# sglang-npu/DeepGEMM_Ascend

Hardware: AMD Instinct MI355X
Metric: fp8 TFLOPS + % MFMA peak, 4096^3 block-scaled GEMM; grouped-GEMM tok/s at 1/2/4/8 GPU (higher is better)
Workload: dtype bf16

## Files before the change

### deepgemm_ascend_amd/__init__.py

```python
from ._lib import DGAError, DGALibraryError, Platform, Problem, Tiling, build, lib
from .api import (
    CONFIG_FIELDS,
    bbit_params,
    bench_params_fill,
    catlass_dynamic_matmul,
    combine_tokens,
    combine_tokens_weight_grad,
    copy_rows,
    copy_rows2,
    gather_per_token_cast_to_fp8_transposed,
    gemm_fp8_fp8_bf16_nt,
    gemm_fp8_fp8_fp32_nt,
    tiling_check_fp32_out,
    tiling_fp32_out,
    tiling_check_wgrad,
    tiling_wgrad,
    wgrad_gemm_fp8_fp8_fp32_nt,
    k_grouped_wgrad_gemm_fp8_fp8_fp32_nt,
    tiling_check_k_grouped_wgrad,
    tiling_k_grouped_wgrad,
    gemm_fp8_loop_clock,
    get_bench_config,
    get_best_config,
    infer_dtype,
    infer_shape,
    get_m_alignment_for_contiguous_layout,
    m_grouped_gemm_fp8_fp8_bf16_nt_contiguous,
    m_grouped_gemm_fp8_fp8_bf16_nt_masked,
    m_grouped_gemm_fp8_fp8_bf16_nt_masked_indexed,
    mfma_ceiling,
    per_block_cast_to_fp8,
    per_block_cast_to_fp8_transposed,
    per_token_cast_to_fp8,
    per_token_cast_to_fp8_transposed,
    platform_ascend910b,
    predict_time_us,
    route_slots,
    router_topk,
    router_topk_backward,
    route_tokens,
    predictor_load,
    predictor_loaded,
    predictor_unload,
    release_scratch,
    select_kernel_with_predictor,
    select_tiling_strategy,
    silu_and_mul_per_token_cast_to_fp8,
    silu_and_mul_per_token_cast_to_fp8_transposed,
    silu_and_mul_backward_per_token_cast_to_fp8,
    platform_mi355x,
    run_mmad_bench,
    run_mmad_custom,
    run_mmad_rtc,
    select_kernel,
    tiling,
    tiling_check,
    tiling_cache_clear,
    tiling_cache_open,
    tiling_cache_size,
    workspace_bytes,
)
# ... 3 lines not shown
```

### deepgemm_ascend_amd/_lib.py

```python
from __future__ import annotations

import ctypes
import os
import subprocess
from ctypes import POINTER, c_char_p, c_float, c_int, c_int32, c_int64, c_size_t, c_uint8, c_uint16, c_uint32, c_uint64, c_void_p
from pathlib import Path

_PKG = Path(__file__).resolve().parent
LIB_PATH = _PKG / "libdga_hip.so"


class DGALibraryError(RuntimeError):
    pass


class DGAError(RuntimeError):

    def __init__(self, status: int, where: str, detail: str = ""):
        self.status = status
        msg = f"{where}: status {status} ({status_string(status)})"
        if detail:
            msg += f" {detail}"
        super().__init__(msg)

# ... 109 lines not shown
    "dga_cast_to_fp8_128x128": (c_int, [c_void_p, c_int, c_int64, c_int64, c_void_p, c_void_p, c_void_p]),
    "dga_cast_to_fp8_1x128_ld": (c_int, [c_void_p, c_int, c_int64, c_int64, c_void_p, c_int64, c_void_p, c_void_p]),
    "dga_cast_to_fp8_128x128_ld": (c_int, [c_void_p, c_int, c_int64, c_int64, c_void_p, c_int64, c_void_p, c_void_p]),
    "dga_cast_to_fp8_1x128_ex": (c_int, [c_void_p, c_int, c_int64, c_int64, c_void_p, c_int64, c_void_p, c_int, c_void_p]),
    "dga_cast_to_fp8_128x128_ex": (c_int, [c_void_p, c_int, c_int64, c_int64, c_void_p, c_int64, c_void_p, c_int, c_void_p]),
    "dga_silu_mul_cast_to_fp8_1x128": (c_int, [c_void_p, c_int, c_int64, c_int64, c_int64, c_void_p, c_void_p, c_void_p, c_void_p, c_int,
                                       c_void_p]),
    "dga_silu_mul_bwd_cast_to_fp8_1x128": (c_int, [c_void_p, c_void_p, c_int, c_int64, c_int64, c_int64, c_void_p, c_void_p, c_void_p,
                                           c_void_p, c_void_p, c_int, c_void_p]),
    "dga_cast_to_fp8_1x128_transposed": (c_int, [c_void_p, c_int, c_int64, c_int64, c_int64, c_void_p, c_void_p, c_void_p, c_int64,
                                         c_void_p, c_void_p, c_void_p, c_int, c_void_p]),
    "dga_silu_mul_cast_to_fp8_1x128_transposed": (c_int, [c_void_p, c_int, c_int64, c_int64, c_int64, c_void_p, c_void_p, c_void_p, c_int64,
                                                  c_void_p, c_void_p, c_void_p, c_int, c_void_p]),
    "dga_cast_to_fp8_128x128_transposed": (c_int, [c_void_p, c_int, c_int64, c_int64, c_int64, c_void_p, c_void_p, c_void_p, c_void_p, c_int,
                                           c_void_p]),
    "dga_gather_cast_to_fp8_1x128_transposed": (c_int, [c_void_p, c_int, c_int64, c_int64, c_void_p, c_int64, c_void_p, c_int64, c_int64,
                                                c_void_p, c_void_p, c_int64, c_void_p, c_void_p, c_void_p, c_int, c_void_p]),
    "dga_combine_rows": (c_int, [c_void_p, c_int, c_int64, c_int64, c_void_p, c_void_p, c_int64, c_int64, c_void_p, c_int, c_void_p]),
    "dga_combine_rows_weight_grad": (c_int, [c_void_p, c_void_p, c_int, c_int64, c_int64, c_void_p, c_int64, c_int64, c_void_p, c_void_p]),
    "dga_router_topk": (c_int, [c_void_p, c_int, c_int64, c_int64, c_int64, c_int, c_void_p, c_int64, c_int64, c_int, c_float, c_void_p, c_void_p,
                                c_void_p, c_void_p]),
    "dga_router_topk_backward": (c_int, [c_void_p, c_void_p, c_void_p, c_int64, c_int64, c_int64, c_int, c_int, c_float, c_void_p, c_int,
                                         c_void_p]),
    "dga_catlass_dynamic_matmul_workspace_bytes": (c_size_t, [c_int, c_int, c_int, c_void_p, c_void_p]),
    "dga_catlass_dynamic_matmul": (c_int, [c_void_p, c_void_p, c_void_p, c_int, c_int, c_int, c_int, c_void_p, c_size_t,
                                           c_void_p]),
    "dga_get_best_config": (c_int, [c_uint32] * 4 + [POINTER(c_uint32)]),
    "dga_get_bench_config": (c_int, [c_uint32] * 9 + [POINTER(c_uint32)]),
    "dga_bench_params_fill": (c_int, [c_uint32] * 3 + [POINTER(c_int32)]),
    "dga_bbit_params": (c_int, [c_uint32] * 9 + [POINTER(c_uint32)]),
    "dga_run_mmad_rtc": (c_int, [c_void_p, c_void_p, c_void_p, c_int, c_int, c_int, c_int, c_int, c_void_p]),
    "dga_run_mmad_bench": (c_int, [c_void_p, c_void_p, c_void_p, c_int, c_int, c_int, c_int, POINTER(c_int32),
                                   c_void_p]),
    "dga_mmad_workspace_bytes": (c_size_t, [c_int, c_int, c_int, c_int, c_void_p]),
    "dga_run_mmad_rtc_ws": (c_int, [c_void_p, c_void_p, c_void_p, c_int, c_int, c_int, c_int, c_int, c_void_p, c_size_t,
                                    c_void_p]),
    "dga_run_mmad_bench_ws": (c_int, [c_void_p, c_void_p, c_void_p, c_int, c_int, c_int, c_int, POINTER(c_int32),
                                      c_void_p, c_size_t, c_void_p]),
    "dga_route_tokens": (c_int, [c_void_p, c_int64, c_int, c_void_p, c_void_p, c_void_p]),
    "dga_route_slots": (c_int, [c_void_p, c_int64, c_int64, c_int, c_int, c_int, c_int, c_int, c_void_p, c_int, c_void_p,
                                c_void_p, c_int64, c_void_p, c_void_p, c_int64, c_void_p]),
    "dga_m_grouped_gemm_fp8_fp8_bf16_nt_masked_indexed": (c_int, [c_void_p, c_int64, c_void_p, c_int64, c_void_p, c_void_p,
                                                                  c_void_p, c_int64, c_void_p, c_int64, c_void_p, c_int,
                                                                  c_int, c_int, c_int, c_int, POINTER(Tiling), c_void_p,
                                                                  c_size_t, c_void_p]),
    "dga_copy_rows2": (c_int, [c_void_p, c_int64, c_void_p, c_int64, c_int64, c_void_p, c_int64, c_void_p, c_int64, c_int64,
# ... 81 lines not shown
```

### deepgemm_ascend_amd/api.py

```python
from __future__ import annotations

import ctypes
import os
from typing import Optional, Sequence, Tuple

import torch

from . import _lib
from ._lib import DGAError, Platform, Problem, Tiling

_FP8 = getattr(torch, "float8_e4m3fn", None)


_raw_stream = getattr(torch._C, "_cuda_getCurrentRawStream", None)


def _stream_of(index: int) -> int:
    if _raw_stream is not None:
        return _raw_stream(index)
    return torch.cuda.current_stream(index).cuda_stream


def _stream_ptr(t: torch.Tensor) -> int:
    if t.is_cuda:
# ... 614 lines not shown
    if masked_m.dtype != torch.int32 or masked_m.dim() != 1 or masked_m.shape[0] != g:
        _fail("masked_m must be int32 [G]")
    if not (a.is_contiguous() and b.is_contiguous() and sfa.is_contiguous() and sfb.is_contiguous() and out.is_contiguous() and
            masked_m.is_contiguous()):
        _fail("operands must be contiguous")
    expected_m = int(expected_m)
    with _device_guard(a, b, sfa, sfb, out, masked_m):
        index = out.device.index
        if tiling_ is None:
            tiling_ = _planned(index, mmax, n, k, g, expected_m, False, strict, policy)
        else:
            tiling_ = _with_policy(tiling_, strict, policy)
        stream = _stream_of(index)
        ws_ptr, ws_bytes = _workspace(tiling_, out.device, stream)
        rc = _lib.lib().dga_m_grouped_gemm_fp8_fp8_bf16_nt_masked(
            a.data_ptr(), sfa.data_ptr(), b.data_ptr(), sfb.data_ptr(), out.data_ptr(), masked_m.data_ptr(),
            g, mmax, n, k, expected_m, ctypes.byref(tiling_), ws_ptr, ws_bytes, stream)
        if rc:
            _lib.check(rc, "m_grouped_gemm_fp8_fp8_bf16_nt_masked")
        if sync:
            torch.cuda.current_stream(out.device).synchronize()


def m_grouped_gemm_fp8_fp8_bf16_nt_masked_indexed(a_rows: torch.Tensor, sfa_src: torch.Tensor, sfa_byte_offset: int,
                                                  sfa_ld: int, rhs, out_rows: torch.Tensor, row_index: torch.Tensor,
                                                  masked_m: torch.Tensor, m_max: int, expected_m: int = 0,
                                                  tiling_: Optional[Tiling] = None, sync: bool = False,
                                                  strict: bool = False, policy: Optional[str] = None) -> None:
    b, sfb = rhs
    _fp8_bytes(b); _fp8_bytes(a_rows)
    _require(a_rows.dim() == 2 and a_rows.stride(1) == 1 and out_rows.dim() == 2 and out_rows.stride(1) == 1, "2-D row tensors")
    g, n, k = b.shape
    rows, lda = a_rows.shape[0], a_rows.stride(0)
    kb, nb = (k + 127) // 128, (n + 127) // 128
    _require(a_rows.shape[1] >= k and out_rows.shape[1] >= n and out_rows.dtype == torch.bfloat16, "row widths")
    _require(out_rows.shape[0] >= rows, "out_rows must have a row for every source row")
    _require(tuple(sfb.shape) == (g, nb, kb) and sfb.dtype == torch.float32, f"sfb must be [{g},{nb},{kb}] f32")
    _require(row_index.dtype == torch.int64 and row_index.numel() >= g * m_max and row_index.is_contiguous(), "row_index int64[G*m_max]")
    _require(masked_m.dtype == torch.int32 and tuple(masked_m.shape) == (g,), "masked_m must be int32 [G]")
    _require(sfa_byte_offset % 4 == 0 and sfa_ld >= kb, "scale rows must be float-aligned")
    _require(sfa_src.dim() == 2 and sfa_src.stride(1) == 1 and sfa_src.dtype in (torch.float32, torch.uint8),
             "sfa_src must be a 2-D float32 (or uint8 payload) row tensor with unit inner stride")
    _require(sfa_src.stride(0) * sfa_src.element_size() == 4 * sfa_ld, "sfa_ld must be sfa_src's row stride in floats")
    _require(sfa_src.data_ptr() % 4 == 0 and sfa_src.shape[0] >= rows and
             sfa_byte_offset + 4 * kb <= sfa_src.shape[1] * sfa_src.element_size(),
             "sfa_src must hold ceil(K/128) floats at sfa_byte_offset of each of the source's rows")
# ... 532 lines not shown
```

### deepgemm_ascend_amd/csrc/dga_fp8_menu.hpp

```cpp
#pragma once
#include "dga_internal.hpp"
#include "gemm_fp8_kernel.hpp"

namespace dga {

template <class Cfg, int PP, bool CLK = false>
int launch_cfg(const GemmParams &p, hipStream_t stream);

#define DGA_MENU_A(X) X(256, 256, 4, 2, 2, 0) X(256, 256, 4, 2, 2, 1) X(256, 256, 4, 2, 2, 2)
#define DGA_MENU_B(X)                                                                                              \
    X(128, 256, 2, 2, 2, 2) X(256, 128, 4, 1, 2, 2) X(128, 128, 2, 2, 2, 2) X(64, 256, 1, 4, 2, 2) X(128, 256, 2, 4, 2, 2)
#define DGA_MENU_C(X)                                                                                              \
    X(128, 256, 2, 2, 2, 0) X(256, 128, 4, 1, 2, 0) X(128, 128, 2, 2, 2, 0) X(64, 256, 1, 4, 2, 0) X(64, 128, 1, 4, 2, 0) \
    X(128, 256, 2, 4, 2, 0) X(128, 256, 2, 4, 3, 0) X(128, 256, 2, 2, 3, 0) X(128, 128, 2, 2, 3, 0) X(64, 256, 1, 4, 3, 0) \
    X(32, 256, 1, 4, 2, 0) X(32, 128, 1, 4, 2, 0) X(16, 256, 1, 4, 2, 0) X(16, 128, 1, 4, 2, 0)                        \
    X(64, 128, 1, 4, 3, 0) X(32, 256, 1, 4, 3, 0) X(32, 128, 1, 4, 3, 0) X(16, 256, 1, 4, 3, 0) X(16, 128, 1, 4, 3, 0)
#define DGA_MENU_LC(X) X(128, 256, 2, 2, 3, 0) X(128, 128, 2, 2, 3, 0) X(64, 256, 1, 4, 3, 0) X(64, 128, 1, 4, 3, 0) X(16, 128, 1, 4, 3, 0)
#define DGA_MENU_CLK(X) X(256, 256, 4, 2, 2, 2)
#define DGA_MENU_CLK_LC(X) X(128, 256, 2, 2, 3, 0)

#define DGA_MENU_EXTERN(BM, BN, WM, WN, ST, PP) \
    extern template int launch_cfg<GemmCfg<BM, BN, WM, WN, ST>, PP, false>(const GemmParams &, hipStream_t);
#define DGA_MENU_EXTERN_CLK(BM, BN, WM, WN, ST, PP) \
    extern template int launch_cfg<GemmCfg<BM, BN, WM, WN, ST>, PP, true>(const GemmParams &, hipStream_t);
// ... 20 lines not shown
#define DGA_MENU_EXTERN_BX(BM, BN, WM, WN, ST, PP) \
    extern template int launch_bf16x<GemmCfg<BM, BN, WM, WN, ST>>(const GemmParams &, hipStream_t);
DGA_MENU_BX(DGA_MENU_EXTERN_BX)
template <class Cfg>
int launch_bf16x_f32(const GemmParams &p, hipStream_t stream);
#define DGA_MENU_EXTERN_BX_F32(BM, BN, WM, WN, ST, PP) \
    extern template int launch_bf16x_f32<GemmCfg<BM, BN, WM, WN, ST>>(const GemmParams &, hipStream_t);
DGA_MENU_BX(DGA_MENU_EXTERN_BX_F32)
template <class Cfg>
int launch_bf16x_rows(const GemmParams &p, hipStream_t stream);
#define DGA_MENU_EXTERN_BX_ROWS(BM, BN, WM, WN, ST, PP) \
    extern template int launch_bf16x_rows<GemmCfg<BM, BN, WM, WN, ST>>(const GemmParams &, hipStream_t);
DGA_MENU_BX(DGA_MENU_EXTERN_BX_ROWS)

int launch_bf16x_image(const GemmParams &p, int waves, hipStream_t stream);
int launch_bf16x_persistent(const GemmParams &p, Out out, hipStream_t stream);
template <class Cfg>
int launch_bf16x_kgroup(const GemmParams &p, hipStream_t stream);
#define DGA_MENU_EXTERN_BX_KGROUP(BM, BN, WM, WN, ST, PP) \
    extern template int launch_bf16x_kgroup<GemmCfg<BM, BN, WM, WN, ST>>(const GemmParams &, hipStream_t);
DGA_MENU_BX(DGA_MENU_EXTERN_BX_KGROUP)
int launch_bf16x_persistent_kgroup(const GemmParams &p, hipStream_t stream);
int launch_strict_kgroup(const GemmParams &p, int bm, hipStream_t stream);
int launch_bf16x_grouped(const GemmParams &p, hipStream_t stream);

int launch_unaligned(const GemmParams &p, hipStream_t stream);

int launch_wsk(const GemmParams &p, hipStream_t stream);
int launch_wsk_dma(const GemmParams &p, hipStream_t stream, int math = 0, Out out = Out::Bf16);
int wsk_rows(int m);
int wsk_max_ntiles(int m);

int launch_ue8m0(int bm, int bn, bool loaders, bool cont, const GemmParams &p, hipStream_t stream);
int launch_ue8m0_w4(const GemmParams &p, hipStream_t stream);
int launch_bf16u(int bm, int bn, const GemmParams &p, hipStream_t stream);

int launch_streamk(const GemmParams &p, void *ws, size_t ws_bytes, bool ue8m0, hipStream_t stream);
size_t streamk_workspace_bytes();
int launch_bf16x_streamk(const GemmParams &p, void *ws, size_t ws_bytes, hipStream_t stream, Out out = Out::Bf16);
size_t bx_streamk_workspace_bytes();
int coresident_workgroups(hipStream_t stream);
int launch_bf16x_dsk(const GemmParams &p, int splits, void *ws, size_t ws_bytes, hipStream_t stream, Out out = Out::Bf16);
int bx_dsk_splits(int64_t tiles, int kb, int want, int cus);
size_t bx_dsk_workspace_bytes(int64_t tiles, int splits);

int launch_cont_persistent(const GemmParams &p, hipStream_t stream);

// ... 2 lines not shown
```

### deepgemm_ascend_amd/csrc/dga_internal.hpp

```cpp
#pragma once
#include <hip/hip_runtime_api.h>

#include "dga_hip.h"
#include <cstdint>
#include <cstdlib>

namespace dga {
int record_hip(hipError_t e);
uint32_t device_cus();
int default_policy();
struct Fp8Indexed {
    const int64_t *row_index;
    int64_t lda;
    int64_t sfa_ld;
    int64_t ldc;
    int64_t rows;
};
struct Fp8Strided {
    int64_t lda, ldb;
    int flags;
};
enum class Out { Bf16, F32, F32Rows };
struct Fp8Call {
    const void *a;
// ... 10 lines not shown
    const int32_t *masked_m = nullptr;
    const int32_t *m_indices = nullptr;
    const Fp8Indexed *ix = nullptr;
    const Fp8Strided *sd = nullptr;
    Out kind = Out::Bf16;
    const float *c_in = nullptr;
    unsigned long long *clock_stamps = nullptr;
};
int run_fp8(const Fp8Call &c);
inline int env_int(const char *name, int dflt)
{
    const char *e = std::getenv(name);
    return e ? std::atoi(e) : dflt;
}
int variant_count();
void variant_info(int i, int *bm, int *bn, int *wm, int *wn, int *lds);
int variant_stages(int i);
bool variant_has_loader_waves(int i);
void prefer_loader_waves(dga_tiling_t &t, bool upgrade_plain = true);
int pad_rows(const void *src0, void *dst0, int64_t rows0, const void *src1, void *dst1, int64_t rows1, int64_t src_row_bytes,
             int64_t dst_row_bytes, hipStream_t stream);
int pad_rows_strided(const void *src0, int64_t stride0, void *dst0, int64_t rows0, const void *src1, int64_t stride1, void *dst1,
                     int64_t rows1, int64_t src_row_bytes, int64_t dst_row_bytes, hipStream_t stream);
void apply_tail_split(dga_tiling_t &t, uint32_t cus);
}
```

### deepgemm_ascend_amd/csrc/dga_launch.hip

```cpp
#include <hip/hip_runtime.h>
#include <atomic>
#include <cstdio>
#include <cstdlib>
#include <cstring>
#include <mutex>

#include "dga_hip.h"
#include "dga_internal.hpp"
#include "dga_fp8_menu_impl.hpp"
#include "gemm_fp8_aux_kernels.hpp"

namespace dga {

static std::atomic<int> g_last_hip_error{0};
int record_hip(hipError_t e)
{
    if (e != hipSuccess) {
        g_last_hip_error.store(static_cast<int>(e));
        return DGA_E_HIP;
    }
    return DGA_OK;
}
uint32_t device_cus()
{
// ... 426 lines not shown
        if (tail > 0 && tail * 2 <= cus && main_tiles > 0 && vq && vq->bm == 64 && vq->bn == 128) {
            GemmParams pm = p;
            pm.launch_tiles = main_tiles;
            rc = launch_bf16x_persistent(pm, c.kind, c.stream);
            if (rc == DGA_E_TILING) rc = vx->launch[form](pm, c.stream);
            if (rc != DGA_OK) return rc;
            GemmParams pt = p;
            pt.tail_begin = main_tiles;
            pt.tail_sub = 2;
            pt.launch_tiles = tail * 4;
            return vq->launch[form](pt, c.stream);
        }
    }
    const int64_t tiles = static_cast<int64_t>(p.groups) * p.tiles_m * p.tiles_n, cus = static_cast<int64_t>(device_cus());
    if (t.kernelSerial == DGA_KERNEL_STREAMK_ONE_LAUNCH && vx->bm == 128 && vx->bn == 256 && dense && c.kind != Out::F32Rows) {
        const size_t need = bx_streamk_workspace_bytes();
        if (uint8_t *sk_ws = carve(need)) {
            rc = launch_bf16x_streamk(p, sk_ws, need, c.stream, c.kind);
            if (rc != DGA_E_TILING) return rc;
        }
    }
    if (vx->bm == 128 && vx->bn == 256 && !c.m_indices && c.kind == Out::Bf16 &&
        (env().bx_grouped >= 0 ? (env().bx_grouped != 0 && c.masked_m) : t.build == DGA_BUILD_BX_GROUPED)) {
        rc = launch_bf16x_grouped(p, c.stream);
        if (rc != DGA_E_TILING) return rc;
    }
    const bool pays = tiles > cus;
    if (vx->bm == 128 && vx->bn == 256 &&
        (env().bx_persist >= 0 ? env().bx_persist != 0 : (t.build == DGA_BUILD_BX_PERSISTENT || (t.build != DGA_BUILD_BX_ONE_TILE && pays)))) {
        rc = launch_bf16x_persistent(p, c.kind, c.stream);
        if (rc != DGA_E_TILING) return rc;
    }
    return vx->launch[form](p, c.stream);
}

static int run_fast(const Fp8Call &c, const dga_tiling_t &t, const Variant *v, bool ue8m0, GemmParams &p, Carver &carve)
{
    const bool dense = c.groups == 1 && !c.masked_m && !c.m_indices && !c.ix;
    const hipStream_t stream = c.stream;
    if (!c.clock_stamps && dense && (env().wsk >= 0 ? env().wsk != 0 : t.kernelSerial == DGA_KERNEL_SPLITK_WORKGROUP)) {
        if (env().wsk_dma >= 0 ? env().wsk_dma != 0 : t.build != DGA_BUILD_WSK_REGISTER) {
            const int rc = launch_wsk_dma(p, stream);
            if (rc != DGA_E_TILING) return rc;
        }
        const int rc = launch_wsk(p, stream);
        if (rc != DGA_E_TILING) return rc;
    }
// ... 374 lines not shown
```

### deepgemm_ascend_amd/csrc/dga_launch_menu_l.hip

```cpp
#include <cstdlib>
#include "dga_fp8_menu_impl.hpp"
#include "gemm_fp8_bf16x_grouped_kernel.hpp"
namespace dga {

template <bool KTAIL, bool BNT, bool STAG, bool IDX = false>
static int launch_bf16x_grouped_one(const GemmParams &p, hipStream_t stream)
{
    typedef GemmCfg<128, 256, 2, 4, 3> Cfg;
    constexpr int kLds = Cfg::LDS_BYTES + (IDX ? 256 * 16 : 0);
    const int64_t tiles = static_cast<int64_t>(p.groups) * p.tiles_m * p.tiles_n;
    const unsigned grid = static_cast<unsigned>(std::min<int64_t>(tiles, device_cus()));
    return launch_kernel<gemm_fp8_bf16x_grouped_kernel<KTAIL, BNT, STAG, IDX>>(grid, Cfg::NT, kLds, stream, p);
}

int launch_bf16x_grouped(const GemmParams &p, hipStream_t stream)
{
    if (p.tail_sub || p.m_indices || p.launch_tiles > 0 || p.splitk > 1 || p.kb_n < 2) return DGA_E_TILING;
    const bool nt = p.b_nt != 0;
#ifdef DGA_BXG_KNOBS
    if (const char *e = std::getenv("DGA_BXG_KNOB"); e && (std::atoi(e) & 2)) {
        if (p.k % 128) return nt ? launch_bf16x_grouped_one<true, true, false>(p, stream) : launch_bf16x_grouped_one<true, false, false>(p, stream);
        return nt ? launch_bf16x_grouped_one<false, true, false>(p, stream) : launch_bf16x_grouped_one<false, false, false>(p, stream);
    }
#endif
    if (p.row_index) {
        if (p.k % 128) return nt ? launch_bf16x_grouped_one<true, true, true, true>(p, stream) : launch_bf16x_grouped_one<true, false, true, true>(p, stream);
        return nt ? launch_bf16x_grouped_one<false, true, true, true>(p, stream) : launch_bf16x_grouped_one<false, false, true, true>(p, stream);
    }
    if (p.k % 128) return nt ? launch_bf16x_grouped_one<true, true, true>(p, stream) : launch_bf16x_grouped_one<true, false, true>(p, stream);
    return nt ? launch_bf16x_grouped_one<false, true, true>(p, stream) : launch_bf16x_grouped_one<false, false, true>(p, stream);
}
}
```

### deepgemm_ascend_amd/csrc/dga_tiling.cpp

```cpp
#include <dlfcn.h>

#include <algorithm>
#include <cmath>
#include <cstdint>
#include <cstdio>
#include <cstdlib>
#include <cstring>
#include <fstream>
#include <map>
#include <mutex>
#include <sstream>
#include <string>
#include <tuple>
#include <vector>

#include "dga_hip.h"
#include "dga_internal.hpp"

namespace dga {
namespace tiling {

inline uint32_t ceil_div(uint32_t a, uint32_t b) { return (a + b - 1) / b; }
inline uint32_t round_up(uint32_t v, uint32_t al) { return ceil_div(v, al) * al; }

// ... 988 lines not shown
}

int dga_tiling_cache_open(const char *csv_path) { return Cache::instance().open(csv_path); }
int dga_tiling_cache_clear(void) { Cache::instance().clear(); return DGA_OK; }
int dga_tiling_cache_size(void) { return Cache::instance().size(); }

size_t dga_workspace_bytes(const dga_tiling_t *tiling)
{
    if (!tiling) return 0;
    size_t bytes = 0;
    auto add = [&](size_t b) { bytes = ((bytes + 255) & ~size_t(255)) + b; };
    const size_t groups = tiling->groups ? tiling->groups : 1;
    if (tiling->k % 16 != 0 && tiling->k > 0) {
        const size_t kp = (static_cast<size_t>(tiling->k) + 127) / 128 * 128;
        add((tiling->contiguous ? 1 : groups) * tiling->m * kp);
        add(groups * tiling->n * kp);
    }
    if (tiling->splitkFactor > 1) add(static_cast<size_t>(tiling->splitkFactor) * tiling->m * tiling->n * 4);
    if (tiling->kernelSerial == DGA_KERNEL_STREAMK_ONE_LAUNCH) add(static_cast<size_t>(dga::device_cus()) * (256 * 256 * 4 + 8) + 256);
    if (tiling->build == DGA_BUILD_BX_DECODE && tiling->splitkFactor > 1) {
        const size_t tiles = (static_cast<size_t>(tiling->m) + 63) / 64 * ((static_cast<size_t>(tiling->n) + 127) / 128);
        add(tiles * (tiling->splitkFactor - 1) * (64 * 128 * 4 + 8) + 256);
    }
    return bytes ? bytes + 256 : 0;
}

const char *dga_status_string(int status)
{
    switch (status) {
        case DGA_OK: return "ok";
        case DGA_E_NULL: return "null pointer";
        case DGA_E_SHAPE: return "shape / rank / layout mismatch";
        case DGA_E_DTYPE: return "dtype mismatch";
        case DGA_E_ALIGN: return "alignment";
        case DGA_E_HIP: return "HIP runtime error";
        case DGA_E_TILING: return "no compiled kernel for this tiling";
        case DGA_E_WORKSPACE: return "workspace too small";
        case DGA_E_IO: return "file error";
        case DGA_E_RANGE: return "value out of range";
        default: return "unknown";
    }
}

int dga_abi_version(void) { return DGA_ABI_VERSION; }

}
// ... 1 lines not shown
```

### deepgemm_ascend_amd/csrc/gemm_fp8_bf16x_grouped_kernel.hpp

```cpp
#pragma once
#include "gemm_fp8_kernel.hpp"

namespace dga {

template <bool KTAIL, bool BNT, bool STAGGER = true, bool INDEXED = false>
__global__ void __launch_bounds__(512) __attribute__((amdgpu_waves_per_eu(2, 2)))
gemm_fp8_bf16x_grouped_kernel(const GemmParams p)
{
    typedef GemmCfg<128, 256, 2, 4, 3> Cfg;
    constexpr int BM = Cfg::kBM, BN = Cfg::kBN, WN = Cfg::kWN, TM = Cfg::TM, TN = Cfg::TN, DNT = Cfg::DNT;
    constexpr int NL = Cfg::LOADS_PER_STAGE, LAGT = 2, RING = 4, NT = Cfg::NT;
    static_assert(Cfg::NT == 512 && DNT == 512 && TM == 4 && TN == 4 && Cfg::SC_ITERS == 1 && Cfg::STAGES == 3, "the grouped schedule");
    typedef __bf16 v8bf __attribute__((ext_vector_type(8)));
    extern __shared__ __attribute__((aligned(16))) uint8_t smem[];

    const int tid = threadIdx.x, lane = tid & 63;
    const int wave = __builtin_amdgcn_readfirstlane(tid >> 6);
    const int wm = wave / WN, wn = wave % WN;
    const int li = lane & 15, kg = lane >> 4;
    const int KB = p.kb_n;

    const int tiles_per_group = p.tiles_m * p.tiles_n;
    const int total = p.groups * tiles_per_group;
    int first = 0, count = total, step = gridDim.x, slot = blockIdx.x;
    if (p.xcd_remap) {
        const int xcd = blockIdx.x & 7, q = total >> 3, r = total & 7;
        first = xcd < r ? xcd * (q + 1) : r * (q + 1) + (xcd - r) * q;
        count = q + (xcd < r ? 1 : 0);
        step = ((int)gridDim.x - xcd + 7) >> 3;
        slot = blockIdx.x >> 3;
    }
    struct Tile { int g, M, m0, n0; };
    typedef const __attribute__((address_space(4))) int32_t *const_i32_ptr;
    const const_i32_ptr masked_m_c = (const_i32_ptr)p.masked_m;
    auto seek = [&](int &local, Tile &t) -> bool {
        for (; local < count; local += step) {
            const int tile = first + local;
            const int g = tile / tiles_per_group;
            const int t_in = tile - g * tiles_per_group;
            const int gm = p.raster_group;
            const int per = gm * p.tiles_n;
            const int band = t_in / per;
            const int row0 = band * gm;
            const int rows = min(p.tiles_m - row0, gm);
            const int loc = t_in - band * per;
            const int tm = row0 + loc % rows, tn = loc / rows;
            const int M = p.masked_m ? min(masked_m_c[g], p.m) : p.m;
            const int m0 = tm * BM;
            if (m0 >= M) continue;
            t.g = g; t.M = M; t.m0 = m0; t.n0 = tn * BN;
            return true;
        }
        return false;
    };

    const uint32_t lds0 = (uint32_t)(uintptr_t)(lptr_t)smem;
    constexpr uint32_t kOutOfRange = 0x80000000u;
    const int a_col = ((tid & 7) ^ swz_a(tid >> 3)) * 16;
    const int b_col = ((tid & 7) ^ swz_b(tid >> 3)) * 16;
    v4i a_rsrc, b_rsrc;
    uint32_t a_voff[Cfg::A_ITERS], b_voff[Cfg::B_ITERS];
    const float *sc_src;
    int kbf = 0;
    bool fill_valid = true;
    constexpr bool indexed = INDEXED;
    static_assert(Cfg::A_ITERS == 2, "partner slot: two A offsets and the scale pointer");
    uint32_t *const pslot = reinterpret_cast<uint32_t *>(smem + Cfg::LDS_BYTES) + (tid & (DNT / 2 - 1)) * 4;
    auto a_off_of = [&](const Tile &t, int it, int td) -> uint32_t {
        const int row = (it * DNT + td) >> 3;
        if (row >= t.M - t.m0) return kOutOfRange;
// ... 337 lines not shown
```

### deepgemm_ascend_amd/csrc/gemm_fp8_kernel.hpp

```cpp
#pragma once
#include "dga_device_common.hpp"
#include "dga_hip.h"

namespace dga {

struct GemmParams {
    const uint8_t *a;
    const float *sfa;
    const uint8_t *b;
    const float *sfb;
    uint16_t *out;
    union {
        const int32_t *masked_m;
        const int32_t *ks;
    };
    const int32_t *m_indices;
    const int64_t *row_index;
    int64_t sfa_ld;
    int64_t a_bytes;
    int b_groups;
    int m;
    int n, k, kb_n, nb_n;
    int64_t lda, ldb, ldc;
    int64_t a_gs, b_gs, c_gs;
    int64_t sfa_gs, sfb_gs;
    int tiles_m, tiles_n, groups;
    int raster_group;
    int xcd_remap;
    union {
        float *partial;
        const float *c_in;
    };
    int splitk, kb_per_split;
    int b_nt;
    int out_nt;
    int launch_tiles;
    int tail_begin, tail_sub;
    unsigned long long *stamps;
};

__device__ __forceinline__ float add_c_no_fma(float v, float c)
{
#pragma clang fp contract(off)
    return v + c;
}
__device__ __forceinline__ v4f add_c_no_fma(v4f v, v4f c)
{
#pragma clang fp contract(off)
    return v + c;
}
__device__ __forceinline__ void store_f32x4(float *dst, v4f v, int out_nt)
{
    if (out_nt == 1) asm volatile("global_store_dwordx4 %0, %1, off nt" :: "v"(dst), "v"(v) : "memory");
    else if (out_nt == 2) asm volatile("global_store_dwordx4 %0, %1, off sc0 sc1" :: "v"(dst), "v"(v) : "memory");
    else if (out_nt == 3) asm volatile("global_store_dwordx4 %0, %1, off sc0 sc1 nt" :: "v"(dst), "v"(v) : "memory");
    else *(v4f *)dst = v;
}
template <int W>
__device__ __forceinline__ void store_row_f32(float *orow, const float *crow, int n, int N, bool vec, int out_nt, const v4f (&v)[W / 4])
{
    if (vec && n + W <= N) {
// ... 1094 lines not shown
```

### include/dga_hip.h

```cpp
#ifndef DGA_HIP_H
#define DGA_HIP_H

#include <stddef.h>
#include <stdint.h>

#ifdef __cplusplus
extern "C" {
#endif

#define DGA_ABI_VERSION 7

enum {
    DGA_OK = 0,
    DGA_E_NULL = -1,
    DGA_E_SHAPE = -2,
    DGA_E_DTYPE = -3,
    DGA_E_ALIGN = -4,
    DGA_E_HIP = -5,
    DGA_E_TILING = -6,
    DGA_E_WORKSPACE = -7,
    DGA_E_IO = -8,
    DGA_E_RANGE = -9
};

// ... 120 lines not shown
                             size_t workspace_bytes, void *stream);

int dga_wgrad_gemm_fp8_fp8_fp32_nt(const void *a, int64_t lda, const float *sfa, const void *b, int64_t ldb, const float *sfb,
                                   const float *c, float *out, int m, int n, int k, int flags, const dga_tiling_t *tiling,
                                   void *workspace, size_t workspace_bytes, void *stream);

int dga_k_grouped_wgrad_gemm_fp8_fp8_fp32_nt(const void *a, int64_t lda, const float *sfa, const void *b, int64_t ldb, const float *sfb,
                                             const float *c, float *out, const int32_t *ks, int groups, int m, int n, int k_total,
                                             int flags, const dga_tiling_t *tiling, void *workspace, size_t workspace_bytes,
                                             void *stream);

int dga_m_grouped_gemm_fp8_fp8_bf16_nt_masked(const void *a, const float *sfa, const void *b, const float *sfb,
                                              void *out, const int32_t *masked_m, int groups, int m_max, int n,
                                              int k, int expected_m, const dga_tiling_t *tiling, void *workspace,
                                              size_t workspace_bytes, void *stream);

int dga_m_grouped_gemm_fp8_fp8_bf16_nt_masked_indexed(const void *a, int64_t lda, const float *sfa, int64_t sfa_ld,
                                                      const void *b, const float *sfb, void *out, int64_t ldc,
                                                      const int64_t *row_index, int64_t rows, const int32_t *masked_m,
                                                      int groups, int m_max, int n, int k, int expected_m,
                                                      const dga_tiling_t *tiling, void *workspace, size_t workspace_bytes,
                                                      void *stream);

size_t dga_catlass_dynamic_matmul_workspace_bytes(int m, int n, int k, const void *self, const void *mat2);
int dga_catlass_dynamic_matmul(const void *self, const void *mat2, void *out, int m, int n, int k, int dtype,
                               void *workspace, size_t workspace_bytes, void *stream);

int dga_m_grouped_gemm_fp8_fp8_bf16_nt_contiguous(const void *a, const float *sfa, const void *b, const float *sfb,
                                                  void *out, const int32_t *m_indices, int m_sum, int groups, int n,
                                                  int k, const dga_tiling_t *tiling, void *workspace,
                                                  size_t workspace_bytes, void *stream);

int dga_cast_to_fp8_1x128(const void *x, int x_dtype, int64_t rows, int64_t k, void *q, float *sf, void *stream);
int dga_cast_to_fp8_128x128(const void *x, int x_dtype, int64_t rows, int64_t k, void *q, float *sf, void *stream);
int dga_cast_to_fp8_1x128_ld(const void *x, int x_dtype, int64_t rows, int64_t k, void *q, int64_t ldq, float *sf, void *stream);
int dga_cast_to_fp8_128x128_ld(const void *x, int x_dtype, int64_t rows, int64_t k, void *q, int64_t ldq, float *sf, void *stream);
#define DGA_CAST_UE8M0 1
int dga_cast_to_fp8_1x128_ex(const void *x, int x_dtype, int64_t rows, int64_t k, void *q, int64_t ldq, float *sf, int flags, void *stream);
int dga_cast_to_fp8_128x128_ex(const void *x, int x_dtype, int64_t rows, int64_t k, void *q, int64_t ldq, float *sf, int flags, void *stream);

int dga_silu_mul_cast_to_fp8_1x128(const void *x, int x_dtype, int64_t groups, int64_t rows, int64_t h,
                                   const int32_t *masked_m, const int32_t *m_indices,
                                   void *q, float *sf, int flags, void *stream);

int dga_silu_mul_bwd_cast_to_fp8_1x128(const void *x, const void *grad_h, int dtype, int64_t groups, int64_t rows, int64_t h,
                                       const int32_t *masked_m, const int32_t *m_indices,
// ... 159 lines not shown
```

Before: 1215.

## Reorder masked grouped-GEMM experts by workload to balance XCD/CU assignment

Adds a small pre-kernel that ranks experts by estimated tile work from masked_m and builds a permutation table, dealt across XCD bins in a serpentine order. The masked grouped kernel gains an ORDERED variant that reads the group id and clamped row count from this table, so heavy experts are spread evenly across the persistent CTAs and XCDs. This targets load imbalance when masked_m varies per expert. It costs an extra tiny kernel launch and a workspace carve per call, is enabled by default through an environment switch, and includes a host reference implementation plus Python bindings.

```diff
diff --git a/deepgemm_ascend_amd/__init__.py b/deepgemm_ascend_amd/__init__.py
--- a/deepgemm_ascend_amd/__init__.py
+++ b/deepgemm_ascend_amd/__init__.py
@@ -37,6 +37,9 @@
     predict_time_us,
     route_slots,
     router_topk,
+    set_grouped_order,
+    grouped_order_reference,
+    grouped_order_table,
     router_topk_backward,
     route_tokens,
     predictor_load,
diff --git a/deepgemm_ascend_amd/_lib.py b/deepgemm_ascend_amd/_lib.py
--- a/deepgemm_ascend_amd/_lib.py
+++ b/deepgemm_ascend_amd/_lib.py
@@ -155,6 +155,9 @@
                                 c_void_p, c_void_p]),
     "dga_router_topk_backward": (c_int, [c_void_p, c_void_p, c_void_p, c_int64, c_int64, c_int64, c_int, c_int, c_float, c_void_p, c_int,
                                          c_void_p]),
+    "dga_set_grouped_order": (c_int, [c_int]),
+    "dga_grouped_order_reference": (c_int, [c_void_p, c_int, c_int, c_int, c_int, c_int, c_int, c_void_p]),
+    "dga_grouped_order": (c_int, [c_void_p, c_int, c_int, c_int, c_int, c_int, c_int, c_void_p, c_void_p]),
     "dga_catlass_dynamic_matmul_workspace_bytes": (c_size_t, [c_int, c_int, c_int, c_void_p, c_void_p]),
     "dga_catlass_dynamic_matmul": (c_int, [c_void_p, c_void_p, c_void_p, c_int, c_int, c_int, c_int, c_void_p, c_size_t,
                                            c_void_p]),
diff --git a/deepgemm_ascend_amd/api.py b/deepgemm_ascend_amd/api.py
--- a/deepgemm_ascend_amd/api.py
+++ b/deepgemm_ascend_amd/api.py
@@ -660,6 +660,42 @@
             torch.cuda.current_stream(out.device).synchronize()
 
 
+def set_grouped_order(ordered: Optional[bool] = None) -> bool:
+    return bool(_lib.lib().dga_set_grouped_order(-1 if ordered is None else int(bool(ordered))))
+
+
+def _grouped_order_launch(groups: int, m_max: int, n: int, grid: Optional[int]) -> Tuple[int, int, int]:
+    tiles_m, tiles_n = -(-int(m_max) // 128), -(-int(n) // 256)
+    if grid is None:
+        p = _lib.Platform()
+        _lib.check(_lib.lib().dga_device_platform(ctypes.byref(p)), "device_platform")
+        grid = min(int(groups) * tiles_m * tiles_n, int(p.coreNum))
+    return tiles_m, tiles_n, int(grid)
+
+
+def grouped_order_reference(masked_m, m_max: int, n: int, grid: Optional[int] = None, xcd_remap: bool = True):
+    import numpy as np
+    mm = np.ascontiguousarray(np.asarray(masked_m, dtype=np.int32))
+    _require(mm.ndim == 1 and mm.size > 0, "masked_m must be a non-empty vector")
+    tiles_m, tiles_n, grid = _grouped_order_launch(mm.size, m_max, n, grid)
+    order = np.empty(mm.size, np.int32)
+    _lib.check(_lib.lib().dga_grouped_order_reference(mm.ctypes.data, mm.size, int(m_max), tiles_m, tiles_n, grid, int(bool(xcd_remap)),
+                                                      order.ctypes.data), "grouped_order_reference")
+    return order
+
+
+def grouped_order_table(masked_m: torch.Tensor, m_max: int, n: int, grid: Optional[int] = None, xcd_remap: bool = True) -> torch.Tensor:
+    _require(masked_m.is_cuda and masked_m.dtype == torch.int32 and masked_m.dim() == 1 and masked_m.is_contiguous() and
+             masked_m.numel() > 0, "masked_m must be a contiguous int32 vector on the device")
+    with _device_guard(masked_m):
+        g = masked_m.numel()
+        tiles_m, tiles_n, grid = _grouped_order_launch(g, m_max, n, grid)
+        table = torch.empty((g, 2), dtype=torch.int32, device=masked_m.device)
+        _lib.check(_lib.lib().dga_grouped_order(masked_m.data_ptr(), g, int(m_max), tiles_m, tiles_n, grid, int(bool(xcd_remap)),
+                                                table.data_ptr(), _stream_ptr(masked_m)), "grouped_order")
+    return table
+
+
 def m_grouped_gemm_fp8_fp8_bf16_nt_masked_indexed(a_rows: torch.Tensor, sfa_src: torch.Tensor, sfa_byte_offset: int,
                                                   sfa_ld: int, rhs, out_rows: torch.Tensor, row_index: torch.Tensor,
                                                   masked_m: torch.Tensor, m_max: int, expected_m: int = 0,
diff --git a/deepgemm_ascend_amd/csrc/dga_fp8_menu.hpp b/deepgemm_ascend_amd/csrc/dga_fp8_menu.hpp
--- a/deepgemm_ascend_amd/csrc/dga_fp8_menu.hpp
+++ b/deepgemm_ascend_amd/csrc/dga_fp8_menu.hpp
@@ -66,7 +66,9 @@
 DGA_MENU_BX(DGA_MENU_EXTERN_BX_KGROUP)
 int launch_bf16x_persistent_kgroup(const GemmParams &p, hipStream_t stream);
 int launch_strict_kgroup(const GemmParams &p, int bm, hipStream_t stream);
-int launch_bf16x_grouped(const GemmParams &p, hipStream_t stream);
+int launch_bf16x_grouped(const GemmParams &p, int32_t *order_table, hipStream_t stream);
+int launch_group_order(const int32_t *masked_m, int groups, int m, int tiles_m, int tiles_n, int grid, int xcd_remap, int32_t *table,
+                       hipStream_t stream);
 
 int launch_unaligned(const GemmParams &p, hipStream_t stream);
 
diff --git a/deepgemm_ascend_amd/csrc/dga_group_order.hip b/deepgemm_ascend_amd/csrc/dga_group_order.hip
--- /dev/null
+++ b/deepgemm_ascend_amd/csrc/dga_group_order.hip
@@ -0,0 +1,168 @@
+#include <hip/hip_runtime.h>
+#include <stdint.h>
+
+#include <algorithm>
+#include <numeric>
+#include <vector>
+
+#include "dga_fp8_menu.hpp"
+
+namespace dga {
+
+struct OrderWalk {
+    int experts;
+    int bins0, more;
+    __host__ __device__ int bins(int x) const { return bins0 + (x < more ? 1 : 0); }
+};
+
+__host__ __device__ inline bool order_walk(int groups, int tiles_per_group, int grid, int xcd_remap, OrderWalk &w)
+{
+    if (!xcd_remap || groups < 8 || (groups & 7) || groups > kGroupOrderMaxGroups || tiles_per_group < 1 || grid < 8) return false;
+    const int step = grid >> 3, more = grid & 7;
+    if (step % tiles_per_group || (more && tiles_per_group > 1)) return false;
+    w.experts = groups >> 3;
+    w.bins0 = step / tiles_per_group;
+    w.more = more;
+    return w.bins0 < w.experts;
+}
+
+__host__ __device__ inline int order_rows(int masked, int m) { return masked < 0 ? 0 : (masked < m ? masked : m); }
+
+__host__ __device__ inline int order_weight(int rows, int tiles_m)
+{
+    int w = 0;
+    for (int tm = 0; tm < tiles_m; ++tm) {
+        const int r = rows - 128 * tm;
+        if (r <= 0) break;
+        const int mt = ((r < 128 ? r : 128) + 15) >> 4;
+        w += 4 + mt > 7 ? 4 + mt : 7;
+    }
+    return w;
+}
+
+__host__ __device__ inline int order_rank_of_place(const OrderWalk &w, int place)
+{
+    const int E = w.experts, x = place / E, l = place - x * E;
+    const int b = l % w.bins(x), j = l / w.bins(x);
+    int before = 0, in_round = 0, ahead = 0;
+    for (int y = 0; y < 8; ++y) {
+        const int done = j * w.bins(y) < E ? j * w.bins(y) : E;
+        const int here = E - done < w.bins(y) ? E - done : w.bins(y);
+        before += done;
+        in_round += here;
+        if (y < x) ahead += here;
+    }
+    const int i = ahead + b;
+    return before + ((j & 1) ? in_round - 1 - i : i);
+}
+
+__host__ __device__ inline int order_key(int weight, int expert) { return weight * kGroupOrderMaxGroups + (kGroupOrderMaxGroups - 1 - expert); }
+
+__global__ void __launch_bounds__(1024)
+group_order_kernel(const int32_t *__restrict__ masked_m, int groups, int m, int tiles_m, int tiles_per_group, int grid, int xcd_remap,
+                   int lanes, int2 *__restrict__ table)
+{
+    __shared__ __attribute__((aligned(16))) int key[kGroupOrderMaxGroups];
+    __shared__ int rows_of[kGroupOrderMaxGroups], sorted[kGroupOrderMaxGroups], larger[kGroupOrderMaxGroups];
+    __shared__ int differ;
+    const int tid = threadIdx.x;
+    OrderWalk walk;
+    if (!order_walk(groups, tiles_per_group, grid, xcd_remap, walk)) {
+        for (int e = tid; e < groups; e += blockDim.x) table[e] = make_int2(e, order_rows(masked_m[e], m));
+        return;
+    }
+    if (tid < groups) {
+        const int rows = order_rows(masked_m[tid], m);
+        rows_of[tid] = rows;
+        key[tid] = order_key(order_weight(rows, tiles_m), tid);
+    }
+    if (tid == 0) differ = 0;
+    __syncthreads();
+    const int part = tid / lanes, e = tid - part * lanes, parts = blockDim.x / lanes;
+    const int share = ((groups + parts - 1) / parts + 3) & ~3, f0 = part * share, f1 = f0 + share < groups ? f0 + share : groups;
+    const int my_key = e < groups ? key[e] : 0;
+    int count = 0;
+#pragma unroll 4
+    for (int f = f0; f < f1; f += 4) {
+        const int4 v = *reinterpret_cast<const int4 *>(&key[f]);
+        count += (v.x > my_key ? 1 : 0) + (v.y > my_key ? 1 : 0) + (v.z > my_key ? 1 : 0) + (v.w > my_key ? 1 : 0);
+    }
+    larger[tid] = count;
+    if (tid < groups && my_key / kGroupOrderMaxGroups != key[0] / kGroupOrderMaxGroups) differ = 1;
+    __syncthreads();
+    if (tid < groups) {
+        int rank = 0;
+        for (int q = 0; q < parts; ++q) rank += larger[q * lanes + tid];
+        sorted[rank] = tid;
+    }
+    __syncthreads();
+    if (tid < groups) {
+        const int expert = differ ? sorted[order_rank_of_place(walk, tid)] : tid;
+        table[tid] = make_int2(expert, rows_of[expert]);
+    }
+}
+
+bool group_order_applies(int groups, int tiles_per_group, int grid, int xcd_remap)
+{
+    OrderWalk w;
+    return order_walk(groups, tiles_per_group, grid, xcd_remap, w);
+}
+
+int launch_group_order(const int32_t *masked_m, int groups, int m, int tiles_m, int tiles_n, int grid, int xcd_remap, int32_t *table,
+                       hipStream_t stream)
+{
+    const int tpg = tiles_m * tiles_n;
+    const int lanes = (groups + 63) & ~63;
+    const unsigned threads = group_order_applies(groups, tpg, grid, xcd_remap) ? static_cast<unsigned>(1024 / lanes * lanes) : 256u;
+    hipLaunchKernelGGL(group_order_kernel, dim3(1), dim3(threads), 0, stream, masked_m, groups, m, tiles_m, tpg, grid, xcd_remap, lanes,
+                       reinterpret_cast<int2 *>(table));
+    return record_hip(hipGetLastError());
+}
+
+static int group_order_reference(const int32_t *masked_m, int groups, int m, int tiles_m, int tiles_n, int grid, int xcd_remap, int32_t *order)
+{
+    std::iota(order, order + groups, 0);
+    OrderWalk walk;
+    if (!order_walk(groups, tiles_m * tiles_n, grid, xcd_remap, walk)) return DGA_OK;
+    std::vector<int> weight(groups), sorted(groups);
+    for (int e = 0; e < groups; ++e) weight[e] = order_weight(order_rows(masked_m[e], m), tiles_m);
+    if (std::all_of(weight.begin(), weight.end(), [&](int w) { return w == weight[0]; })) return DGA_OK;
+    std::iota(sorted.begin(), sorted.end(), 0);
+    std::stable_sort(sorted.begin(), sorted.end(), [&](int a, int b) { return weight[a] > weight[b]; });
+    for (int r = 0; r + 1 < groups; ++r)
+        if (order_key(weight[sorted[r]], sorted[r]) <= order_key(weight[sorted[r + 1]], sorted[r + 1])) return DGA_E_RANGE;
+    const int E = walk.experts;
+    int dealt = 0;
+    for (int j = 0; dealt < groups; ++j) {
+        std::vector<int> places;
+        for (int x = 0; x < 8; ++x)
+            for (int b = 0; b < walk.bins(x) && b + j * walk.bins(x) < E; ++b) places.push_back(x * E + b + j * walk.bins(x));
+        if (places.empty()) return DGA_E_RANGE;
+        const int n = static_cast<int>(places.size());
+        for (int i = 0; i < n; ++i) {
+            const int rank = dealt + ((j & 1) ? n - 1 - i : i);
+            if (order_rank_of_place(walk, places[i]) != rank) return DGA_E_RANGE;
+            order[places[i]] = sorted[rank];
+        }
+        dealt += n;
+    }
+    return DGA_OK;
+}
+
+}
+
+extern "C" int dga_grouped_order_reference(const int32_t *masked_m, int groups, int m, int tiles_m, int tiles_n, int grid, int xcd_remap,
+                                           int32_t *order)
+{
+    if (!masked_m || !order) return DGA_E_NULL;
+    if (groups < 1 || m < 0 || tiles_m < 1 || tiles_n < 1 || grid < 1) return DGA_E_SHAPE;
+    return dga::group_order_reference(masked_m, groups, m, tiles_m, tiles_n, grid, xcd_remap, order);
+}
+
+extern "C" int dga_grouped_order(const int32_t *masked_m, int groups, int m, int tiles_m, int tiles_n, int grid, int xcd_remap,
+                                 int32_t *table, void *stream)
+{
+    if (!masked_m || !table) return DGA_E_NULL;
+    if (groups < 1 || m < 0 || tiles_m < 1 || tiles_n < 1 || grid < 1) return DGA_E_SHAPE;
+    return dga::launch_group_order(masked_m, groups, m, tiles_m, tiles_n, grid, xcd_remap, table, static_cast<hipStream_t>(stream));
+}
diff --git a/deepgemm_ascend_amd/csrc/dga_internal.hpp b/deepgemm_ascend_amd/csrc/dga_internal.hpp
--- a/deepgemm_ascend_amd/csrc/dga_internal.hpp
+++ b/deepgemm_ascend_amd/csrc/dga_internal.hpp
@@ -56,5 +56,8 @@
              int64_t dst_row_bytes, hipStream_t stream);
 int pad_rows_strided(const void *src0, int64_t stride0, void *dst0, int64_t rows0, const void *src1, int64_t stride1, void *dst1,
                      int64_t rows1, int64_t src_row_bytes, int64_t dst_row_bytes, hipStream_t stream);
+constexpr int kGroupOrderMaxGroups = 1024;
+constexpr size_t kGroupOrderTableBytes = 8;
+bool group_order_applies(int groups, int tiles_per_group, int grid, int xcd_remap);
 void apply_tail_split(dga_tiling_t &t, uint32_t cus);
 }
diff --git a/deepgemm_ascend_amd/csrc/dga_launch.hip b/deepgemm_ascend_amd/csrc/dga_launch.hip
--- a/deepgemm_ascend_amd/csrc/dga_launch.hip
+++ b/deepgemm_ascend_amd/csrc/dga_launch.hip
@@ -472,7 +472,9 @@
     }
     if (vx->bm == 128 && vx->bn == 256 && !c.m_indices && c.kind == Out::Bf16 &&
         (env().bx_grouped >= 0 ? (env().bx_grouped != 0 && c.masked_m) : t.build == DGA_BUILD_BX_GROUPED)) {
-        rc = launch_bf16x_grouped(p, c.stream);
+        uint8_t *order_table = c.masked_m && c.groups >= 8 && c.groups % 8 == 0 && c.groups <= kGroupOrderMaxGroups
+                                   ? carve(static_cast<size_t>(c.groups) * kGroupOrderTableBytes) : nullptr;
+        rc = launch_bf16x_grouped(p, reinterpret_cast<int32_t *>(order_table), c.stream);
         if (rc != DGA_E_TILING) return rc;
     }
     const bool pays = tiles > cus;
diff --git a/deepgemm_ascend_amd/csrc/dga_launch_menu_l.hip b/deepgemm_ascend_amd/csrc/dga_launch_menu_l.hip
--- a/deepgemm_ascend_amd/csrc/dga_launch_menu_l.hip
+++ b/deepgemm_ascend_amd/csrc/dga_launch_menu_l.hip
@@ -1,33 +1,55 @@
+#include <atomic>
 #include <cstdlib>
 #include "dga_fp8_menu_impl.hpp"
 #include "gemm_fp8_bf16x_grouped_kernel.hpp"
 namespace dga {
 
-template <bool KTAIL, bool BNT, bool STAG, bool IDX = false>
+static std::atomic<int> g_grouped_order{env_int("DGA_GROUPED_ORDER", 1) != 0};
+
+template <bool KTAIL, bool BNT, bool STAG, bool IDX = false, bool ORD = false>
 static int launch_bf16x_grouped_one(const GemmParams &p, hipStream_t stream)
 {
     typedef GemmCfg<128, 256, 2, 4, 3> Cfg;
     constexpr int kLds = Cfg::LDS_BYTES + (IDX ? 256 * 16 : 0);
     const int64_t tiles = static_cast<int64_t>(p.groups) * p.tiles_m * p.tiles_n;
     const unsigned grid = static_cast<unsigned>(std::min<int64_t>(tiles, device_cus()));
-    return launch_kernel<gemm_fp8_bf16x_grouped_kernel<KTAIL, BNT, STAG, IDX>>(grid, Cfg::NT, kLds, stream, p);
+    return launch_kernel<gemm_fp8_bf16x_grouped_kernel<KTAIL, BNT, STAG, IDX, ORD>>(grid, Cfg::NT, kLds, stream, p);
 }
 
-int launch_bf16x_grouped(const GemmParams &p, hipStream_t stream)
+template <bool IDX, bool ORD>
+static int launch_bf16x_grouped_form(const GemmParams &p, hipStream_t stream)
 {
-    if (p.tail_sub || p.m_indices || p.launch_tiles > 0 || p.splitk > 1 || p.kb_n < 2) return DGA_E_TILING;
     const bool nt = p.b_nt != 0;
+    if (p.k % 128) return nt ? launch_bf16x_grouped_one<true, true, true, IDX, ORD>(p, stream) : launch_bf16x_grouped_one<true, false, true, IDX, ORD>(p, stream);
+    return nt ? launch_bf16x_grouped_one<false, true, true, IDX, ORD>(p, stream) : launch_bf16x_grouped_one<false, false, true, IDX, ORD>(p, stream);
+}
+
+int launch_bf16x_grouped(const GemmParams &p0, int32_t *order_table, hipStream_t stream)
+{
+    if (p0.tail_sub || p0.m_indices || p0.launch_tiles > 0 || p0.splitk > 1 || p0.kb_n < 2) return DGA_E_TILING;
+    const bool nt = p0.b_nt != 0;
 #ifdef DGA_BXG_KNOBS
     if (const char *e = std::getenv("DGA_BXG_KNOB"); e && (std::atoi(e) & 2)) {
-        if (p.k % 128) return nt ? launch_bf16x_grouped_one<true, true, false>(p, stream) : launch_bf16x_grouped_one<true, false, false>(p, stream);
-        return nt ? launch_bf16x_grouped_one<false, true, false>(p, stream) : launch_bf16x_grouped_one<false, false, false>(p, stream);
+        if (p0.k % 128) return nt ? launch_bf16x_grouped_one<true, true, false>(p0, stream) : launch_bf16x_grouped_one<true, false, false>(p0, stream);
+        return nt ? launch_bf16x_grouped_one<false, true, false>(p0, stream) : launch_bf16x_grouped_one<false, false, false>(p0, stream);
     }
 #endif
-    if (p.row_index) {
-        if (p.k % 128) return nt ? launch_bf16x_grouped_one<true, true, true, true>(p, stream) : launch_bf16x_grouped_one<true, false, true, true>(p, stream);
-        return nt ? launch_bf16x_grouped_one<false, true, true, true>(p, stream) : launch_bf16x_grouped_one<false, false, true, true>(p, stream);
+    GemmParams p = p0;
+    p.group_order = nullptr;
+    const int64_t tiles = static_cast<int64_t>(p.groups) * p.tiles_m * p.tiles_n;
+    const int grid = static_cast<int>(std::min<int64_t>(tiles, device_cus()));
+    if (p.masked_m && order_table && g_grouped_order.load(std::memory_order_relaxed) &&
+        group_order_applies(p.groups, p.tiles_m * p.tiles_n, grid, p.xcd_remap)) {
+        if (int rc = launch_group_order(p.masked_m, p.groups, p.m, p.tiles_m, p.tiles_n, grid, p.xcd_remap, order_table, stream)) return rc;
+        p.group_order = order_table;
     }
-    if (p.k % 128) return nt ? launch_bf16x_grouped_one<true, true, true>(p, stream) : launch_bf16x_grouped_one<true, false, true>(p, stream);
-    return nt ? launch_bf16x_grouped_one<false, true, true>(p, stream) : launch_bf16x_grouped_one<false, false, true>(p, stream);
+    if (p.group_order) return p.row_index ? launch_bf16x_grouped_form<true, true>(p, stream) : launch_bf16x_grouped_form<false, true>(p, stream);
+    return p.row_index ? launch_bf16x_grouped_form<true, false>(p, stream) : launch_bf16x_grouped_form<false, false>(p, stream);
 }
 }
+
+extern "C" int dga_set_grouped_order(int mode)
+{
+    if (mode < 0) return dga::g_grouped_order.load(std::memory_order_relaxed);
+    return dga::g_grouped_order.exchange(mode != 0, std::memory_order_relaxed);
+}
diff --git a/deepgemm_ascend_amd/csrc/dga_tiling.cpp b/deepgemm_ascend_amd/csrc/dga_tiling.cpp
--- a/deepgemm_ascend_amd/csrc/dga_tiling.cpp
+++ b/deepgemm_ascend_amd/csrc/dga_tiling.cpp
@@ -1034,6 +1034,8 @@
         const size_t tiles = (static_cast<size_t>(tiling->m) + 63) / 64 * ((static_cast<size_t>(tiling->n) + 127) / 128);
         add(tiles * (tiling->splitkFactor - 1) * (64 * 128 * 4 + 8) + 256);
     }
+    if (tiling->build == DGA_BUILD_BX_GROUPED && groups >= 8 && groups % 8 == 0 && groups <= static_cast<size_t>(dga::kGroupOrderMaxGroups))
+        add(groups * dga::kGroupOrderTableBytes);
     return bytes ? bytes + 256 : 0;
 }
 
diff --git a/deepgemm_ascend_amd/csrc/gemm_fp8_bf16x_grouped_kernel.hpp b/deepgemm_ascend_amd/csrc/gemm_fp8_bf16x_grouped_kernel.hpp
--- a/deepgemm_ascend_amd/csrc/gemm_fp8_bf16x_grouped_kernel.hpp
+++ b/deepgemm_ascend_amd/csrc/gemm_fp8_bf16x_grouped_kernel.hpp
@@ -3,7 +3,7 @@
 
 namespace dga {
 
-template <bool KTAIL, bool BNT, bool STAGGER = true, bool INDEXED = false>
+template <bool KTAIL, bool BNT, bool STAGGER = true, bool INDEXED = false, bool ORDERED = false>
 __global__ void __launch_bounds__(512) __attribute__((amdgpu_waves_per_eu(2, 2)))
 gemm_fp8_bf16x_grouped_kernel(const GemmParams p)
 {
@@ -33,11 +33,17 @@
     struct Tile { int g, M, m0, n0; };
     typedef const __attribute__((address_space(4))) int32_t *const_i32_ptr;
     const const_i32_ptr masked_m_c = (const_i32_ptr)p.masked_m;
+    typedef int v2i_t __attribute__((ext_vector_type(2)));
+    typedef const __attribute__((address_space(4))) v2i_t *const_v2i_ptr;
+    const const_v2i_ptr order_c = (const_v2i_ptr)p.group_order;
     auto seek = [&](int &local, Tile &t) -> bool {
         for (; local < count; local += step) {
             const int tile = first + local;
-            const int g = tile / tiles_per_group;
-            const int t_in = tile - g * tiles_per_group;
+            const int place = tile / tiles_per_group;
+            const int t_in = tile - place * tiles_per_group;
+            v2i_t who{place, 0};
+            if constexpr (ORDERED) who = order_c[place];
+            const int g = who.x;
             const int gm = p.raster_group;
             const int per = gm * p.tiles_n;
             const int band = t_in / per;
@@ -45,7 +51,7 @@
             const int rows = min(p.tiles_m - row0, gm);
             const int loc = t_in - band * per;
             const int tm = row0 + loc % rows, tn = loc / rows;
-            const int M = p.masked_m ? min(masked_m_c[g], p.m) : p.m;
+            const int M = ORDERED ? who.y : (p.masked_m ? min(masked_m_c[g], p.m) : p.m);
             const int m0 = tm * BM;
             if (m0 >= M) continue;
             t.g = g; t.M = M; t.m0 = m0; t.n0 = tn * BN;
diff --git a/deepgemm_ascend_amd/csrc/gemm_fp8_kernel.hpp b/deepgemm_ascend_amd/csrc/gemm_fp8_kernel.hpp
--- a/deepgemm_ascend_amd/csrc/gemm_fp8_kernel.hpp
+++ b/deepgemm_ascend_amd/csrc/gemm_fp8_kernel.hpp
@@ -37,6 +37,7 @@
     int launch_tiles;
     int tail_begin, tail_sub;
     unsigned long long *stamps;
+    const int32_t *group_order;
 };
 
 __device__ __forceinline__ float add_c_no_fma(float v, float c)
diff --git a/include/dga_hip.h b/include/dga_hip.h
--- a/include/dga_hip.h
+++ b/include/dga_hip.h
@@ -166,6 +166,12 @@
                                                       const dga_tiling_t *tiling, void *workspace, size_t workspace_bytes,
                                                       void *stream);
 
+int dga_set_grouped_order(int mode);
+int dga_grouped_order_reference(const int32_t *masked_m, int groups, int m, int tiles_m, int tiles_n, int grid, int xcd_remap,
+                                int32_t *order);
+int dga_grouped_order(const int32_t *masked_m, int groups, int m, int tiles_m, int tiles_n, int grid, int xcd_remap, int32_t *table,
+                      void *stream);
+
 size_t dga_catlass_dynamic_matmul_workspace_bytes(int m, int n, int k, const void *self, const void *mat2);
 int dga_catlass_dynamic_matmul(const void *self, const void *mat2, void *out, int m, int n, int k, int dtype,
                                void *workspace, size_t workspace_bytes, void *stream);
```

After: 1212. Within noise of the previous version (-0.2%).
